# brech1/keaki

Hardware: AMD Instinct MI355X
Metric: BN254 G1 scalar-mults/sec on 2^24-point MSM (per GPU) (higher is better)
Workload: dtype u32 limbs, 256-bit Montgomery modular integer (9 x 29-bit lazy limbs in the bucket kernel, 8 x 32 elsewhere)

## Files before the change

keaki_amd/csrc/api.hip:

```cpp
#include "internal.h"

#include <algorithm>
#include <set>
#include <utility>
#include <vector>

using namespace keaki_internal;

struct keaki_hip_srs_g1 {
  const void* d = nullptr;
  size_t n = 0;
  bool owned = false;
  int device = -1;
  std::recursive_mutex mu;
  keaki_hip_ctx* acct = nullptr;
  size_t fk_bytes = 0;
  void* table = nullptr;
  size_t table_bytes = 0;
  int c_table = 0;
  void* fk_hat_s = nullptr;
  int fk_log2d = -1;
};
struct keaki_hip_srs_g2 {
  const void* d = nullptr;
// ... 295 lines not shown
    const size_t lo = pipe.ranges[j].first, m = pipe.ranges[j].second;
    return up.chunk(j, (char*)ctx->io_a.p + lo * 32, (const char*)scalars + lo * 32, m * 32);
  };
  return run(&pipe);
}

#define CTX_GUARD(ctx)                                \
  if (!(ctx)) return KEAKI_ERR_BAD_ARG;               \
  std::lock_guard<std::recursive_mutex> lock_((ctx)->mu);       \
  keaki_internal::DeviceScope dev_((ctx)->device);              \
  if (!dev_.ok) return fail(ctx, KEAKI_ERR_HIP, "hipSetDevice(%d) failed", (ctx)->device)

}

extern "C" {

#ifndef KEAKI_SRC_HASH
#define KEAKI_SRC_HASH "unknown"
#endif
#ifdef KEAKI_DIAG
const char* keaki_hip_version(void) { return "keaki-hip 0.3 (gfx950) DIAGNOSTIC BUILD (diag_row_mask available: not the product) src=" KEAKI_SRC_HASH; }
#else
const char* keaki_hip_version(void) { return "keaki-hip 0.3 (gfx950) src=" KEAKI_SRC_HASH; }
#endif

extern "C++" {
namespace {
void tune_from_env(Tuning& t) {
  auto geti = [](const char* name, long long& out) { const char* e = getenv(name); if (!e || !*e) return false; out = atoll(e); return true; };
  long long v;
  if (geti("KEAKI_MSM_C", v)) t.msm_c = (int)v;
  if (geti("KEAKI_MSM_C_SHARED", v)) t.msm_c_shared = (int)v;
  if (geti("KEAKI_REDUCE_L", v)) t.reduce_l = (int)v;
  if (geti("KEAKI_PART_SHIFT", v)) t.part_shift = (int)v;
  if (geti("KEAKI_ACC_U29", v)) t.acc_u29 = v != 0;
  if (geti("KEAKI_ACC_U29_G2", v)) t.acc_u29_g2 = v != 0;
  if (geti("KEAKI_ACC_NT", v)) t.acc_nt = v != 0;
  if (geti("KEAKI_ACC_PREFETCH", v)) t.acc_prefetch = v != 0;
  if (geti("KEAKI_ACC_IDXQ", v)) t.acc_idxq = v != 0;
  if (geti("KEAKI_CS_MASKED", v)) t.cs_masked = v != 0;
  if (geti("KEAKI_FK_UNIFORM", v)) t.fk_uniform = v != 0;
  if (geti("KEAKI_FK_GTAB", v)) t.fk_gtab = v != 0;
  if (geti("KEAKI_FK_ADDSUB29", v)) t.fk_addsub29 = v != 0;
  if (geti("KEAKI_FK_RADIX4", v)) t.fk_radix4 = v != 0;
  if (geti("KEAKI_FB_OCC1", v)) t.fb_occ1 = v != 0;
  if (geti("KEAKI_MSM_SHORT_TABLES", v)) t.msm_short_tables = (int)v;
  if (geti("KEAKI_PAIR_WIDE_MAX", v)) t.pair_wide_max = (int)v;
  if (geti("KEAKI_PAIR_TWO_WAVES", v)) t.pair_two_waves = v != 0;
  if (geti("KEAKI_GT_WB_B", v)) t.gt_wb_b = (int)v;
  if (geti("KEAKI_ENCAP_GT", v)) t.encap_gt = v;
  if (geti("KEAKI_HOST_PREFAULT", v)) t.host_prefault = v != 0;
  if (geti("KEAKI_PIPE_CHUNKS", v)) t.pipe_chunks = v != 0;
  if (geti("KEAKI_MSM_PIPE_CHUNKS", v)) t.msm_pipe_chunks = (int)v;
  if (geti("KEAKI_MSM_PIPE_MIN", v)) t.msm_pipe_min = v;
  if (geti("KEAKI_MSM_PIPE_GROWTH", v)) t.msm_pipe_growth = (int)v;
}
struct BufClass { DevBuf* b; int cls; };
std::vector<BufClass> all_bufs(keaki_hip_ctx* ctx) {
  std::vector<BufClass> v;
  for (DevBuf* b : {&ctx->digits, &ctx->hist, &ctx->offsets, &ctx->cursor, &ctx->sorted, &ctx->buckets, &ctx->acc29, &ctx->partials, &ctx->wsums, &ctx->bsums,
                    &ctx->tmp_a, &ctx->tmp_b, &ctx->tmp_c, &ctx->io_a, &ctx->io_b, &ctx->io_c, &ctx->io_d, &ctx->io_e, &ctx->perm, &ctx->heavy,
                    &ctx->pair_ws, &ctx->verify_io, &ctx->g2gen_lines, &ctx->fk_tab, &ctx->g2pow_lines, &ctx->g2pow_pts})
    v.push_back({b, 1});
  for (DevBuf* b : {&ctx->fb_bases, &ctx->fb_g1_gen, &ctx->fb_g2_gen, &ctx->fb_com, &ctx->fb_tau, &ctx->gt_tab_a, &ctx->gt_tab_b, &ctx->gt_base,
                    &ctx->fbs_g2_gen, &ctx->fbs_tau, &ctx->fbs_g1_gen})
    v.push_back({b, 2});
// ... 42 lines not shown
  for (const BufClass& bc : all_bufs(ctx))
    if (bc.b->p) (void)hipFree(bc.b->p);
  for (auto& e : ctx->ev) if (e) (void)hipEventDestroy(e);
  for (auto& e : ctx->fk_ev) if (e) (void)hipEventDestroy(e);
  for (auto& e : ctx->pipe_in) if (e) (void)hipEventDestroy(e);
  for (auto& e : ctx->pipe_done) if (e) (void)hipEventDestroy(e);
  for (auto& e : ctx->open_ev) if (e) (void)hipEventDestroy(e);
  if (ctx->copy_stream) { (void)hipStreamSynchronize(ctx->copy_stream); (void)hipStreamDestroy(ctx->copy_stream); }
  for (auto& e : ctx->aux_ev) if (e) (void)hipEventDestroy(e);
  if (ctx->aux_stream) { (void)hipStreamSynchronize(ctx->aux_stream); (void)hipStreamDestroy(ctx->aux_stream); }
  if (ctx->own_stream) (void)hipStreamDestroy(ctx->stream);
  }
  delete ctx;
}

const char* keaki_hip_last_error(const keaki_hip_ctx* ctx) {
  if (!ctx) return g_create_error.c_str();
  thread_local std::string copy;
  keaki_hip_ctx* c = const_cast<keaki_hip_ctx*>(ctx);
  std::lock_guard<std::recursive_mutex> lock_(c->mu);
  copy = c->err;
  return copy.c_str();
}

keaki_status keaki_hip_ctx_set_option(keaki_hip_ctx* ctx, const char* name, int64_t value) {
  if (!ctx) return KEAKI_ERR_BAD_ARG;
  std::lock_guard<std::recursive_mutex> lock_(ctx->mu);
  if (!name) return fail(ctx, KEAKI_ERR_BAD_ARG, "ctx_set_option: name is null");
  Tuning& t = ctx->tune;
  const std::string k(name);
  if (k == "msm_c") t.msm_c = (int)value;
  else if (k == "msm_c_shared") t.msm_c_shared = (int)value;
  else if (k == "reduce_l") t.reduce_l = (int)value;
  else if (k == "part_shift") t.part_shift = (int)value;
  else if (k == "acc_u29") t.acc_u29 = value != 0;
  else if (k == "acc_u29_g2") t.acc_u29_g2 = value != 0;
  else if (k == "acc_nt") t.acc_nt = value != 0;
  else if (k == "acc_prefetch") t.acc_prefetch = value != 0;
  else if (k == "acc_idxq") t.acc_idxq = value != 0;
  else if (k == "cs_masked") t.cs_masked = value != 0;
  else if (k == "fk_uniform") t.fk_uniform = value != 0;
  else if (k == "fk_gtab") t.fk_gtab = value != 0;
  else if (k == "fk_addsub29") t.fk_addsub29 = value != 0;
  else if (k == "fk_radix4") t.fk_radix4 = value != 0;
  else if (k == "fb_occ1") t.fb_occ1 = value != 0;
  else if (k == "msm_short_tables") t.msm_short_tables = (int)value;
  else if (k == "pair_wide_max") t.pair_wide_max = (int)value;
  else if (k == "pair_two_waves") t.pair_two_waves = value != 0;
  else if (k == "gt_wb_b") {
    if (value != 0 && (value < 8 || value > 22 || gt_table_powers((uint32_t)value) > 320)) return fail(ctx, KEAKI_ERR_BAD_ARG, "ctx_set_option: gt_wb_b = %lld out of range", (long long)value);
    if ((int)value != t.gt_wb_b) { ctx->gt_b_ready = false; ctx->gt_b_fallback = false; }
    t.gt_wb_b = (int)value;
  } else if (k == "encap_gt") t.encap_gt = value;
  else if (k == "host_prefault") t.host_prefault = value != 0;
  else if (k == "pipe_chunks") t.pipe_chunks = value != 0;
#ifdef KEAKI_DIAG
  else if (k == "diag_row_mask") t.diag_row_mask = (unsigned)value;
#endif
  else if (k == "msm_pipe_chunks") t.msm_pipe_chunks = (int)value;
  else if (k == "msm_pipe_min") t.msm_pipe_min = value;
  else if (k == "msm_pipe_growth") t.msm_pipe_growth = (int)value;
  else return fail(ctx, KEAKI_ERR_BAD_ARG, "ctx_set_option: unknown option '%s'", name);
  return KEAKI_OK;
}
keaki_status keaki_hip_debug_set_alloc_limit(keaki_hip_ctx* ctx, size_t bytes) {
  if (!ctx) return KEAKI_ERR_BAD_ARG;
// ... 1081 lines not shown
```

keaki_amd/csrc/internal.h:

```cpp
#pragma once
#include <hip/hip_runtime.h>

#include <cstdarg>
#include <cstdio>
#include <cstdlib>
#include <atomic>
#include <cstring>
#include <functional>
#include <mutex>
#include <string>
#include <utility>
#include <vector>

#include "../../include/keaki_hip.h"

namespace keaki_internal {

struct DevBuf {
  void* p = nullptr;
  size_t cap = 0;
};

}

namespace keaki_internal {
struct Tuning {
  int msm_c = 0;
  int msm_c_shared = 0;
  int msm_short_tables = -1;
  int reduce_l = 0;
  int part_shift = -1;
  bool acc_u29 = true;
  bool acc_u29_g2 = true;
  bool acc_prefetch = true;
  bool acc_idxq = true;
  bool cs_masked = true;
  bool acc_nt = false;
  bool fk_uniform = true;
  bool fk_gtab = true;
  bool fk_radix4 = true;
  bool fk_addsub29 = true;
  bool fb_occ1 = false;
  int pair_wide_max = -1;
  bool pair_two_waves = true;
  int gt_wb_b = 0;
  long long encap_gt = -1;
  bool host_prefault = true;
  bool pipe_chunks = true;
  int msm_pipe_chunks = -1;
  long long msm_pipe_min = 1 << 20;
  int msm_pipe_growth = 160;
#ifdef KEAKI_DIAG
  unsigned diag_row_mask = 0;
#endif
  size_t alloc_limit = 0;
};
}

struct keaki_hip_ctx {
  int device = 0;
  uint32_t n_cu = 256;
  keaki_internal::Tuning tune;
  std::atomic<size_t> mem_tables{0};
// ... 151 lines not shown
```

keaki_amd/csrc/msm.hip.h:

```cpp
#pragma once
#include <type_traits>
#include "bn254_curve.hip.h"
#include "fq29.hip.h"
#include "xyzz29.hip.h"
#include "jac29.hip.h"
#include "xyzz29_g2.hip.h"

namespace bn254 {

typedef uint16_t u16;
typedef u32 v4u_t __attribute__((ext_vector_type(4)));
constexpr u32 DIGIT_NONE = 0xFFFFFFFFu;
#ifndef STAMP
#define STAMP(cond, i) do { } while (0)
#endif

struct MsmShape {
  u32 n;
  u32 c;
  u32 W;
  u32 k;
  u32 stride;
};
KDEV u32 msm_width(const MsmShape& s, u32 w) { return w < s.k ? s.c : s.c - 1; }
// ... 1112 lines not shown
  }
  if (l == 0) {
    typename O::P r = sh[0];
    for (u32 k = 0, nd = msm_bit_offset(s, w); k < nd; k++) r = O::dbl(r);
    if (out_jac) store_norm_jac(out_jac, O::store(r));
    else window_sums[w] = O::store(r);
  }
}

template <class F> KDEV Aff<F> xyzz_to_aff_tail(const Xyzz<F>& p) { return xyzz_to_aff(p); }
template <> KDEV Aff<Fq> xyzz_to_aff_tail<Fq>(const Xyzz<Fq>& p) {
  if (xyzz_is_inf(p)) return aff_inf<Fq>();
  Fq izzz = fq_inv(p.zzz);
  Fq izz = fq_sqr(izzz) * fq_sqr(p.zz);
  return {p.x * izz, p.y * izzz};
}
template <class F>
KDEV void store_norm_jac(F* out, const Xyzz<F>& p) {
  Aff<F> a = xyzz_to_aff_tail(p);
  if (xyzz_is_inf(p)) {
    out[0] = f_one<F>(); out[1] = f_one<F>(); out[2] = f_zero<F>();
  } else {
    out[0] = a.x; out[1] = a.y; out[2] = f_one<F>();
  }
}
template <class F>
__global__ void __launch_bounds__(64) k_msm_final(const Xyzz<F>* __restrict__ window_sums, u32 W, F* __restrict__ out_jac) {
  if (threadIdx.x != 0 || blockIdx.x != 0) return;
  Xyzz<F> acc = xyzz_inf<F>();
  for (u32 w = 0; w < W; w++) acc = xyzz_add(acc, window_sums[w]);
  store_norm_jac(out_jac, acc);
}


template <class F>
__global__ void __launch_bounds__(64) k_msm_build_tables(const Aff<F>* __restrict__ points, u32 N, MsmShape s, Aff<F>* __restrict__ table) {
  u32 i = blockIdx.x * blockDim.x + threadIdx.x;
  if (i >= N) return;
  Aff<F> p = points[i];
  table[i] = p;
#pragma unroll 1
  for (u32 w = 1; w < s.W; w++) {
    Jac<F> j = jac_from_aff(p);
    for (u32 d = msm_width(s, w - 1); d > 0; d--) j = jac_dbl(j);
    p = jac_to_aff(j);
    table[(size_t)w * N + i] = p;
  }
}

constexpr u32 TABLE_MAX_W = 16;
static __global__ void __launch_bounds__(64) k_msm_build_tables_g1(const Aff<Fq>* __restrict__ points, u32 N, MsmShape s, Aff<Fq>* __restrict__ table) {
  u32 i = blockIdx.x * blockDim.x + threadIdx.x;
  if (i >= N) return;
  const Aff<Fq> p = points[i];
  table[i] = p;
  if (aff_is_inf(p)) {
    for (u32 w = 1; w < s.W; w++) table[(size_t)w * N + i] = p;
    return;
  }
  J29 j;
  j.x = u29_from_fq(p.x); j.y = u29_from_fq(p.y); j.z = u29_one();
  U29 zs[TABLE_MAX_W];
  U29 prod = u29_one();
#pragma unroll 1
  for (u32 w = 1; w < s.W; w++) {
    for (u32 d = msm_width(s, w - 1); d > 0; d--) j = j29_dbl(j);
// ... 39 lines not shown
```

keaki_amd/csrc/msm_host.hip.h:

```cpp
#pragma once
#include <algorithm>
#include <functional>
#include <type_traits>
#include <vector>
#include "internal.h"
#include "msm.hip.h"

namespace keaki_internal {
using namespace bn254;

inline int choose_window(size_t n, int forced = 0) {
  if (forced >= 3 && forced <= 24) return forced;
  if (n < 32) return 3;
  double best = 1e300;
  int bc = 3;
  for (int c = 3; c <= 22; c++) {
    MsmPlan p = msm_make_plan(n, c);
    if (p.nb > ((size_t)PART_MAX_BINS << PART_MAX_FINE_SHIFT)) continue;
    double cost = (double)n * p.s.W + 2.8 * (double)p.nb;
    if ((double)p.nb < 131072.0) cost *= 131072.0 / (double)p.nb;
    if (cost < best) { best = cost; bc = c; }
  }
  return bc;
}

template <class F>
keaki_status msm_dev(keaki_hip_ctx* ctx, const Aff<F>* d_points, size_t srs_len, const void* d_scalars, size_t n, void* d_out_jac,
                     const Aff<F>* d_table = nullptr, int c_table = 0, const MsmPipe* pipe = nullptr) {
  if (!d_out_jac || (n && (!d_points || !d_scalars))) return fail(ctx, KEAKI_ERR_BAD_ARG, "msm: null pointer");
  if (n > srs_len) return fail(ctx, KEAKI_ERR_TOO_LARGE, "msm: %zu scalars but the SRS holds %zu points", n, srs_len);
  if (n >= (1ull << 31)) return fail(ctx, KEAKI_ERR_BAD_ARG, "msm: n must be < 2^31 per device");
  const bool shared = d_table != nullptr && (n * 2 > srs_len || ctx->tune.msm_short_tables != 0);
  const MsmPlan plan = shared ? msm_make_plan(n, c_table) : msm_make_plan(n, choose_window(n, ctx->tune.msm_c));
  MsmShape s = plan.s;
  MsmShape rs = s;
  size_t nb = plan.nb;
  if (shared) {
    s.stride = (u32)srs_len;
    u32 cr = 0;
    while ((1u << cr) < plan.max_b) cr++;
    rs.n = s.n; rs.c = cr; rs.W = 1; rs.k = 1; rs.stride = 0;
    nb = plan.max_b;
    d_points = d_table;
    if ((double)srs_len * s.W >= 2147483647.0) return fail(ctx, KEAKI_ERR_BAD_ARG, "msm: precomputed table index overflows 31 bits");
  }
  ctx->last_c = (int)s.c;
  if ((double)n * s.W >= 4294967295.0) return fail(ctx, KEAKI_ERR_BAD_ARG, "msm: n * windows overflows 32-bit positions");
  u32 L = sizeof(F) > sizeof(Fq) ? (plan.max_b >= 64 ? 8 : plan.max_b)
                                 : plan.max_b >= (1u << 21) ? 32 : plan.max_b >= (1u << 20) ? 16 : (plan.max_b >= 64 ? 8 : plan.max_b);
  if (ctx->tune.reduce_l >= 1 && ctx->tune.reduce_l <= 4096 && (u32)ctx->tune.reduce_l <= plan.max_b) L = (u32)ctx->tune.reduce_l;
  const u32 chunks = cdiv(plan.max_b, L);
  ST_TRY(reserve(ctx, ctx->wsums, (size_t)rs.W * sizeof(Xyzz<F>)));
  Xyzz<F>* wsums = (Xyzz<F>*)ctx->wsums.p;
  F* out = (F*)d_out_jac;
  hipStream_t st = ctx->stream;
  if (ctx->timing) (void)hipEventRecord(ctx->ev[0], st);
  if (n == 0) {
    hipLaunchKernelGGL((k_msm_final<F>), dim3(1), dim3(64), 0, st, (const Xyzz<F>*)wsums, 0u, out);
    return launch_check(ctx, "msm_final");
  }
  const size_t K = pipe ? pipe->ranges.size() : 1;
  if (pipe && K < 1) return fail(ctx, KEAKI_ERR_BAD_ARG, "msm: bad chunk bounds");
  struct Pass {
    size_t lo, m, pairs, max_chunks, cm_bytes, bt_bytes, bm_bytes, sg_bytes, ts_bytes;
    PartShape ps;
  };
  std::vector<Pass> passes(K);
  size_t w_digits = 0, w_sorted = 0, w_offsets = 0, w_cursor = 0, w_pairs = 0, w_total = 0;
  for (size_t j = 0; j < K; j++) {
    Pass& q = passes[j];
    q.lo = pipe ? pipe->ranges[j].first : 0;
    q.m = pipe ? pipe->ranges[j].second : n;
    if (q.m == 0 || q.lo > n || q.m > n - q.lo) return fail(ctx, KEAKI_ERR_BAD_ARG, "msm: bad chunk bounds");
    w_total += q.m;
    if (!part_make_shape(q.m, s.W, nb, &q.ps, ctx->tune.part_shift))
      return fail(ctx, KEAKI_ERR_BAD_ARG, "msm: %zu buckets / %u windows exceed the bucket sort's LDS budget (window too large)", nb, s.W);
    q.pairs = q.m * (size_t)s.W;
    q.max_chunks = part_max_chunks(q.pairs, q.ps.nbins);
    q.cm_bytes = (size_t)q.ps.nbins * q.ps.ntiles * sizeof(uint2);
    q.bt_bytes = ((size_t)q.ps.nbins * 4 + 15) & ~(size_t)15;
    q.bm_bytes = (size_t)q.ps.nbins * sizeof(BinMeta);
    q.sg_bytes = nb * sizeof(v4u_t);
    q.ts_bytes = (size_t)q.ps.ntiles * (q.ps.nbins + 1) * 2;
    w_digits = std::max(w_digits, (size_t)q.ps.ntiles * q.ps.te * 4);
    w_sorted = std::max(w_sorted, q.pairs * 4 + 64);
    w_offsets = std::max(w_offsets, q.max_chunks * q.ps.nf * 4);
    w_cursor = std::max(w_cursor, q.cm_bytes + q.bt_bytes + q.bm_bytes + q.sg_bytes + q.ts_bytes);
    w_pairs = std::max(w_pairs, q.pairs);
  }
  if (w_total != n) return fail(ctx, KEAKI_ERR_BAD_ARG, "msm: the chunks cover %zu of %zu pairs", w_total, n);
  bool u29 = false;
  if constexpr (std::is_same<F, Fq>::value) u29 = ctx->tune.acc_u29;
  if constexpr (std::is_same<F, Fq2>::value) u29 = ctx->tune.acc_u29_g2;
  bool lazy_state = K > 1 && u29 && std::is_same<F, Fq>::value;
  ST_TRY(reserve(ctx, ctx->digits, w_digits));
  ST_TRY(reserve(ctx, ctx->sorted, w_sorted));
  ST_TRY(reserve(ctx, ctx->hist, nb * 4));
  ST_TRY(reserve(ctx, ctx->offsets, w_offsets));
  ST_TRY(reserve(ctx, ctx->cursor, w_cursor));
  ST_TRY(reserve(ctx, ctx->buckets, nb * sizeof(Xyzz<F>)));
  ST_TRY(reserve(ctx, ctx->partials, ((size_t)rs.W * chunks + (size_t)rs.W * 256) * sizeof(Xyzz<F>)));
  ST_TRY(reserve(ctx, ctx->perm, nb * 4 + 2 * CNT_BINS * 4 + sizeof(HeavyList)));
  const u32 hv_cap = (u32)(w_pairs / HEAVY_MIN + 1), hv_slice_cap = (u32)(hv_cap + w_pairs / HEAVY_SLICE + 1);
  const size_t hv_hdr = ((2 * (size_t)hv_cap + hv_slice_cap) * 4 + 255) & ~(size_t)255;
  ST_TRY(reserve(ctx, ctx->heavy, hv_hdr + (size_t)hv_slice_cap * sizeof(Xyzz<F>)));
  if (lazy_state) {
    const keaki_status st29 = reserve(ctx, ctx->acc29, nb * sizeof(Acc29));
    if (st29 == KEAKI_ERR_OOM) { lazy_state = false; u29 = false; ctx->err.clear(); }
    else if (st29 != KEAKI_OK) return st29;
  }
  u32 *tiles = (u32*)ctx->digits.p, *sorted = (u32*)ctx->sorted.p, *hist = (u32*)ctx->hist.p;
  u32* segoff = (u32*)ctx->offsets.p;
  Xyzz<F>* buckets = (Xyzz<F>*)ctx->buckets.p;
  Xyzz<F>* partials = (Xyzz<F>*)ctx->partials.p;
  Acc29* state29 = lazy_state ? (Acc29*)ctx->acc29.p : nullptr;
  u32* perm = (u32*)ctx->perm.p;
  u32 *gstart = perm + nb, *ghist = gstart + CNT_BINS;
  HeavyList* hv = (HeavyList*)(ghist + CNT_BINS);
  u32 *hv_bucket = (u32*)ctx->heavy.p, *hv_first = hv_bucket + hv_cap, *hv_owner = hv_first + hv_cap;
  Xyzz<F>* hv_slices = (Xyzz<F>*)((char*)ctx->heavy.p + hv_hdr);
  for (size_t j = 0; j < K; j++) {
    const Pass& q = passes[j];
    const PartShape& ps = q.ps;
    if (pipe && pipe->stage) ST_TRY(pipe->stage(j));
    MsmShape sj = s;
    sj.n = (u32)q.m;
    const Fr* scal = (const Fr*)d_scalars + q.lo;
    const Aff<F>* pts = d_points + q.lo;
    const bool first = j == 0, last = j + 1 == K;
    uint2* cellmeta = (uint2*)ctx->cursor.p;
    u32* bin_total = (u32*)((char*)ctx->cursor.p + q.cm_bytes);
    BinMeta* bins = (BinMeta*)((char*)bin_total + q.bt_bytes);
    v4u_t* segtab = (v4u_t*)((char*)bins + q.bm_bytes);
    u16* tstart = (u16*)((char*)segtab + q.sg_bytes);
// ... 48 lines not shown
        if (K == 1) {
          if (ctx->tune.acc_nt) KEAKI_ACC(1, ACC_WHOLE);
          else if (!ctx->tune.acc_prefetch)
            hipLaunchKernelGGL((k_msm_accumulate_g1_u29<0, ACC_WHOLE, 0>), ga, ba, 0, st, pts, view, (const u32*)hist, (const u32*)perm, (u32)nb, buckets, state29);
          else if (!ctx->tune.acc_idxq)
            hipLaunchKernelGGL((k_msm_accumulate_g1_u29<0, ACC_WHOLE, 1>), ga, ba, 0, st, pts, view, (const u32*)hist, (const u32*)perm, (u32)nb, buckets, state29);
          else KEAKI_ACC(0, ACC_WHOLE);
        }
        else if (first) KEAKI_ACC(0, ACC_FIRST);
        else if (!last) KEAKI_ACC(0, ACC_MIDDLE);
        else KEAKI_ACC(0, ACC_LAST);
#undef KEAKI_ACC
        done = true;
      }
    }
    if constexpr (std::is_same<F, Fq2>::value) {
      if (u29) {
        if (first) hipLaunchKernelGGL(k_msm_accumulate_g2_u29<0>, ga, ba, 0, st, pts, view, (const u32*)hist, (const u32*)perm, (u32)nb, buckets);
        else hipLaunchKernelGGL(k_msm_accumulate_g2_u29<1>, ga, ba, 0, st, pts, view, (const u32*)hist, (const u32*)perm, (u32)nb, buckets);
        done = true;
      }
    }
    if (!done)
      hipLaunchKernelGGL((k_msm_accumulate<F>), ga, ba, 0, st, pts, view, (const u32*)hist, (const u32*)perm, (u32)nb, buckets, first ? 0u : 1u);
    ST_TRY(launch_check(ctx, "msm_accumulate"));
    const u32 hv_mode = lazy_state && !last ? (first ? HV_SET29 : HV_ADD29) : (first ? HV_SET : HV_ADD);
    hipLaunchKernelGGL((k_msm_heavy<F>), dim3(HEAVY_GRID), dim3(256), 0, st, pts, view, (const u32*)hist,
                       (const HeavyList*)hv, hv_slice_cap, (const u32*)hv_bucket, (const u32*)hv_first, (const u32*)hv_owner, hv_slices);
    hipLaunchKernelGGL((k_msm_heavy_combine<F>), dim3(HEAVY_COMBINE_GRID), dim3(64), 0, st, (const u32*)hist, (const HeavyList*)hv, hv_cap, hv_slice_cap,
                       (const u32*)hv_bucket, (const u32*)hv_first, (const Xyzz<F>*)hv_slices, buckets, hv_mode, state29);
    ST_TRY(launch_check(ctx, "msm_heavy"));
  }
  if (ctx->timing) (void)hipEventRecord(ctx->ev[2], st);
  hipLaunchKernelGGL((k_msm_reduce<F>), dim3(cdiv((size_t)rs.W * chunks, 64)), dim3(64), 0, st, (const Xyzz<F>*)buckets, rs, L, chunks, partials);
  const Xyzz<F>* fin_in = partials;
  u32 fin_chunks = chunks;
  if (chunks > 256) {
    const u32 G = cdiv(chunks, 128);
    const u32 chunks2 = cdiv(chunks, G);
    Xyzz<F>* partials2 = partials + (size_t)rs.W * chunks;
    hipLaunchKernelGGL((k_msm_partial_groups<F>), dim3(chunks2, rs.W), dim3(64), 0, st, (const Xyzz<F>*)partials, chunks, G, chunks2, partials2);
    fin_in = partials2; fin_chunks = chunks2;
  }
  hipLaunchKernelGGL((k_msm_window_finish<F>), dim3(rs.W), dim3(64), 0, st, fin_in, rs, fin_chunks, wsums, rs.W == 1 ? out : (F*)nullptr);
  if (rs.W != 1) hipLaunchKernelGGL((k_msm_final<F>), dim3(1), dim3(64), 0, st, (const Xyzz<F>*)wsums, rs.W, out);
  ST_TRY(launch_check(ctx, "msm_reduce/final"));
  if (ctx->timing) {
    (void)hipEventRecord(ctx->ev[3], st);
    ctx->timing_pending = true;
  }
  return KEAKI_OK;
}

template <class F>
keaki_status msm_build_tables(keaki_hip_ctx* ctx, const Aff<F>* d_points, size_t N, int c_table, Aff<F>* d_table) {
  MsmPlan plan = msm_make_plan(N, c_table);
  bool done = false;
  if constexpr (std::is_same<F, Fq>::value) {
    if (plan.s.W <= TABLE_MAX_W) {
      hipLaunchKernelGGL(k_msm_build_tables_g1, dim3(cdiv(N, 64)), dim3(64), 0, ctx->stream, d_points, (u32)N, plan.s, d_table);
      done = true;
    }
  }
  if (!done)
  hipLaunchKernelGGL((k_msm_build_tables<F>), dim3(cdiv(N, 64)), dim3(64), 0, ctx->stream, d_points, (u32)N, plan.s, d_table);
  return launch_check(ctx, "msm_build_tables");
// ... 18 lines not shown
```

Baseline: 1.040 billion.

## Replace G1 MSM bucket reduction tail with hierarchical scan and cooperative final sum

Adds a new G1 MSM tail that replaces the per-window reduce, partial-group, window-finish and final kernels. Buckets are summed per chunk as running sums, combined in shared-memory tree groups into per-bit records, and then turned into weighted terms. The terms are doubled by window offset using an 8-lane cooperative XYZZ add/double, and the last block, chosen through an atomic counter, sums them into the output. The aim is to cut serial work and kernel launches in the tail and to spread the per-window doublings and final sum across many threads. The cost is more synchronisation, extra scratch memory, and a last-block reduction pattern that relies on threadfence ordering.

```diff
diff --git a/keaki_amd/csrc/api.hip b/keaki_amd/csrc/api.hip
--- a/keaki_amd/csrc/api.hip
+++ b/keaki_amd/csrc/api.hip
@@ -351,6 +351,7 @@
   if (geti("KEAKI_MSM_C", v)) t.msm_c = (int)v;
   if (geti("KEAKI_MSM_C_SHARED", v)) t.msm_c_shared = (int)v;
   if (geti("KEAKI_REDUCE_L", v)) t.reduce_l = (int)v;
+  if (geti("KEAKI_MSM_TAIL", v)) t.msm_tail = (int)v;
   if (geti("KEAKI_PART_SHIFT", v)) t.part_shift = (int)v;
   if (geti("KEAKI_ACC_U29", v)) t.acc_u29 = v != 0;
   if (geti("KEAKI_ACC_U29_G2", v)) t.acc_u29_g2 = v != 0;
@@ -459,6 +460,7 @@
   if (k == "msm_c") t.msm_c = (int)value;
   else if (k == "msm_c_shared") t.msm_c_shared = (int)value;
   else if (k == "reduce_l") t.reduce_l = (int)value;
+  else if (k == "msm_tail") t.msm_tail = (int)value;
   else if (k == "part_shift") t.part_shift = (int)value;
   else if (k == "acc_u29") t.acc_u29 = value != 0;
   else if (k == "acc_u29_g2") t.acc_u29_g2 = value != 0;
diff --git a/keaki_amd/csrc/internal.h b/keaki_amd/csrc/internal.h
--- a/keaki_amd/csrc/internal.h
+++ b/keaki_amd/csrc/internal.h
@@ -29,6 +29,7 @@
   int msm_c_shared = 0;
   int msm_short_tables = -1;
   int reduce_l = 0;
+  int msm_tail = 1;
   int part_shift = -1;
   bool acc_u29 = true;
   bool acc_u29_g2 = true;
diff --git a/keaki_amd/csrc/msm.hip.h b/keaki_amd/csrc/msm.hip.h
--- a/keaki_amd/csrc/msm.hip.h
+++ b/keaki_amd/csrc/msm.hip.h
@@ -1168,6 +1168,211 @@
   store_norm_jac(out_jac, acc);
 }
 
+constexpr u32 TAILW_SLOTS = 16;
+KDEV void x29w_add(bool act, u32 tl, const X29* A, const X29* B, X29* out, U29* scr) {
+  const bool both = act && !A->inf && !B->inf;
+  if (both && tl < 6) {
+    const U29& p = tl == 0 ? A->x : tl == 1 ? B->x : tl == 2 ? A->y : tl == 3 ? B->y : tl == 4 ? A->zz : A->zzz;
+    const U29& q = tl == 0 ? B->zz : tl == 1 ? A->zz : tl == 2 ? B->zzz : tl == 3 ? A->zzz : tl == 4 ? B->zz : B->zzz;
+    scr[tl] = u29_mul(p, q);
+  }
+  __syncthreads();
+  U29 P, R, U1;
+  bool slow = false;
+  if (both) {
+    U1 = scr[0];
+    P = u29_sub(scr[1], U1, Q29::K8);
+    R = u29_sub(scr[3], scr[2], Q29::K8);
+    slow = u29_maybe_zero(P) && u29_is_zero(P);
+    if (tl < 2) {
+      const U29 o = tl == 0 ? P : R;
+      scr[6 + tl] = u29_mul(o, o);
+    }
+  }
+  __syncthreads();
+  if (both && tl < 3) {
+    const U29 a = tl == 0 ? P : tl == 1 ? U1 : scr[4];
+    scr[8 + tl] = u29_mul(a, scr[6]);
+  }
+  __syncthreads();
+  U29 X3;
+  if (both) {
+    X3 = u29_sub3(scr[7], scr[8], scr[9]);
+    const U29 T = u29_sub_raw(scr[9], X3, Q29::K16);
+    if (tl < 3) {
+      const U29 a = tl == 0 ? scr[5] : tl == 1 ? scr[2] : R;
+      const U29 b = tl == 2 ? T : scr[8];
+      scr[11 + tl] = u29_mul(a, b);
+    }
+  }
+  __syncthreads();
+  if (act && tl == 0) {
+    X29 r;
+    if (A->inf) r = *B;
+    else if (B->inf) r = *A;
+    else if (slow) r = x29_add(*A, *B);
+    else {
+      r.x = X3;
+      r.y = u29_sub(scr[13], scr[12], Q29::K2);
+      r.zz = scr[10];
+      r.zzz = scr[11];
+      r.inf = 0;
+    }
+    *out = r;
+  }
+  __syncthreads();
+}
+KDEV void x29w_dbl(bool act, u32 tl, const X29* A, X29* out, U29* scr) {
+  const bool live = act && !A->inf;
+  U29 U;
+  if (live) {
+    U29 t;
+#pragma unroll
+    for (int i = 0; i < 9; i++) t.l[i] = A->y.l[i] << 1;
+    U = u29_carry(t);
+    if (tl < 2) {
+      const U29 o = tl == 0 ? U : A->x;
+      scr[tl] = u29_mul(o, o);
+    }
+  }
+  __syncthreads();
+  U29 M;
+  if (live) {
+    U29 t;
+#pragma unroll
+    for (int i = 0; i < 9; i++) t.l[i] = 3u * scr[1].l[i];
+    M = u29_carry(t);
+    if (tl < 4) {
+      const U29 a = tl == 0 ? U : tl == 1 ? A->x : tl == 2 ? M : scr[0];
+      const U29 b = tl == 2 ? M : tl == 3 ? A->zz : scr[0];
+      scr[2 + tl] = u29_mul(a, b);
+    }
+  }
+  __syncthreads();
+  U29 X3;
+  if (live) {
+    U29 t;
+#pragma unroll
+    for (int i = 0; i < 9; i++) t.l[i] = scr[4].l[i] - 2u * scr[3].l[i] + Q29::K16W[i];
+    X3 = u29_carry(t);
+    const U29 T = u29_sub_raw(scr[3], X3, Q29::K32);
+    if (tl < 3) {
+      const U29 a = tl == 0 ? M : scr[2];
+      const U29 b = tl == 0 ? T : tl == 1 ? A->y : A->zzz;
+      scr[6 + tl] = u29_mul(a, b);
+    }
+  }
+  __syncthreads();
+  if (act && tl == 0 && live) {
+    X29 r;
+    r.x = X3;
+    r.y = u29_sub(scr[6], scr[7], Q29::K4);
+    r.zz = scr[5];
+    r.zzz = scr[8];
+    r.inf = 0;
+    *out = r;
+  }
+  __syncthreads();
+}
+constexpr u32 TAIL_GROUP_BITS = 8;
+constexpr u32 TAIL_THREADS = 256;
+
+template <class F>
+__global__ void __launch_bounds__(64) k_msm_tail_chunks(const Xyzz<F>* __restrict__ buckets, MsmShape s, u32 lb, u32 chunks_per_window,
+                                                        Xyzz<F>* __restrict__ runs, Xyzz<F>* __restrict__ wss, u32* __restrict__ counter) {
+  const u32 g = blockIdx.x * blockDim.x + threadIdx.x;
+  if (g == 0) *counter = 0;
+  if (g >= s.W * chunks_per_window) return;
+  const u32 w = g / chunks_per_window, t = g % chunks_per_window;
+  const u32 L = 1u << lb, lo = t << lb;
+  const u32 Bw = msm_nbuckets(s, w);
+  const Xyzz<F>* bk = buckets + msm_bucket_base(s, w);
+  typedef TailOps<F> O;
+  typename O::P run = O::inf(), ws = O::inf();
+  for (u32 j = L; j-- > 0;) {
+    if (lo + j < Bw) {
+      run = O::add(run, O::load(bk[lo + j]));
+      ws = O::add(ws, run);
+    }
+  }
+  runs[g] = O::store(run);
+  wss[g] = O::store(ws);
+}
+
+template <class F>
+__global__ void __launch_bounds__(TAIL_THREADS) k_msm_tail_groups(const Xyzz<F>* __restrict__ runs, const Xyzz<F>* __restrict__ wss, u32 chunks_per_window,
+                                                                  u32 gb, Xyzz<F>* __restrict__ rec) {
+  typedef TailOps<F> O;
+  __shared__ typename O::P sh[2 * TAIL_THREADS];
+  const u32 w = blockIdx.y, x = blockIdx.x, l = threadIdx.x;
+  const u32 G = 1u << gb;
+  const size_t t0 = (size_t)w * chunks_per_window + ((size_t)x << gb);
+  if (l < G) {
+    sh[2 * l] = O::load(wss[t0 + l]);
+    sh[2 * l + 1] = O::load(runs[t0 + l]);
+  }
+  __syncthreads();
+  for (u32 d = 0; d < gb; d++) {
+    const u32 nn = G >> (d + 1), half = 1u << (d + 1);
+    const u32 nadd = nn * (d + 2);
+    typename O::P r = O::inf(), c = O::inf();
+    u32 slot = 0, cslot = 0;
+    if (l < nadd) {
+      const u32 k = l / nn, n = l % nn;
+      slot = (n << (d + 2)) + k;
+      r = O::add(sh[slot], sh[slot + half]);
+    }
+    if (l < nn) {
+      cslot = (l << (d + 2));
+      c = sh[cslot + half + 1];
+    }
+    __syncthreads();
+    if (l < nadd) sh[slot] = r;
+    if (l < nn) sh[cslot + d + 2] = c;
+    __syncthreads();
+  }
+  if (l < gb + 2) rec[((size_t)w * gridDim.x + x) * (gb + 2) + l] = O::store(sh[l]);
+}
+
+KDEV void tail_tree(X29* sh, U29* scr, u32 l) {
+  for (u32 h = TAIL_THREADS / 2; h > 8; h >>= 1) {
+    if (l < h) sh[l] = x29_add(sh[l], sh[l + h]);
+    __syncthreads();
+  }
+  const u32 team = l >> 3;
+  for (u32 h = 8; h > 0; h >>= 1) x29w_add(team < h, l & 7, sh + team, sh + team + h, sh + team, scr + (team < 8 ? team : 0) * TAILW_SLOTS);
+}
+
+static __global__ void __launch_bounds__(TAIL_THREADS) k_msm_tail_terms(const Xyzz<Fq>* __restrict__ rec, MsmShape s, u32 lb, u32 gb, u32 gpw,
+                                                                       Xyzz<Fq>* __restrict__ terms, u32* __restrict__ counter, Fq* __restrict__ out_jac) {
+  __shared__ X29 sh[TAIL_THREADS];
+  __shared__ U29 scr[8 * TAILW_SLOTS];
+  __shared__ u32 last;
+  const u32 o = blockIdx.x, w = blockIdx.y, l = threadIdx.x, nt = gridDim.x;
+  const u32 k = o == 0 ? 0u : o <= gb ? o + 1 : 1u;
+  X29 acc = x29_inf();
+  for (u32 x = l; x < gpw; x += TAIL_THREADS)
+    if (o <= gb || ((x >> (o - 1 - gb)) & 1)) acc = x29_add(acc, x29_load(rec[((size_t)w * gpw + x) * (gb + 2) + k]));
+  sh[l] = acc;
+  __syncthreads();
+  tail_tree(sh, scr, l);
+  for (u32 e = msm_bit_offset(s, w) + (o == 0 ? 0u : lb + o - 1); e > 0; e--) x29w_dbl(l < 8, l & 7, sh, sh, scr);
+  if (l == 0) {
+    terms[(size_t)w * nt + o] = x29_store(sh[0]);
+    __threadfence();
+    last = atomicAdd(counter, 1u) == nt * gridDim.y - 1 ? 1u : 0u;
+  }
+  __syncthreads();
+  if (!last) return;
+  __threadfence();
+  acc = x29_inf();
+  for (u32 i = l; i < nt * gridDim.y; i += TAIL_THREADS) acc = x29_add(acc, x29_load(terms[i]));
+  sh[l] = acc;
+  __syncthreads();
+  tail_tree(sh, scr, l);
+  if (l == 0) store_norm_jac(out_jac, x29_store(sh[0]));
+}
+
 
 template <class F>
 __global__ void __launch_bounds__(64) k_msm_build_tables(const Aff<F>* __restrict__ points, u32 N, MsmShape s, Aff<F>* __restrict__ table) {
diff --git a/keaki_amd/csrc/msm_host.hip.h b/keaki_amd/csrc/msm_host.hip.h
--- a/keaki_amd/csrc/msm_host.hip.h
+++ b/keaki_amd/csrc/msm_host.hip.h
@@ -22,6 +22,25 @@
     if (cost < best) { best = cost; bc = c; }
   }
   return bc;
+}
+
+struct TailShape {
+  u32 lb, cpw, gb, gpw, hb, nt;
+  size_t points(u32 W) const { return 2 * (size_t)W * cpw + (size_t)W * gpw * (gb + 2) + (size_t)W * nt + 1; }
+};
+inline TailShape tail_make_shape(u32 W, u32 max_b) {
+  TailShape t;
+  u32 mb = 1, lmb = 0;
+  while (mb < max_b) { mb <<= 1; lmb++; }
+  t.lb = 0;
+  while (t.lb < 4 && t.lb < lmb && (size_t)W * (mb >> t.lb) > (1u << 17)) t.lb++;
+  t.cpw = mb >> t.lb;
+  const u32 lc = lmb - t.lb;
+  t.gb = lc < TAIL_GROUP_BITS ? lc : TAIL_GROUP_BITS;
+  t.hb = lc - t.gb;
+  t.gpw = 1u << t.hb;
+  t.nt = 1 + t.gb + t.hb;
+  return t;
 }
 
 template <class F>
@@ -99,7 +118,9 @@
   ST_TRY(reserve(ctx, ctx->offsets, w_offsets));
   ST_TRY(reserve(ctx, ctx->cursor, w_cursor));
   ST_TRY(reserve(ctx, ctx->buckets, nb * sizeof(Xyzz<F>)));
-  ST_TRY(reserve(ctx, ctx->partials, ((size_t)rs.W * chunks + (size_t)rs.W * 256) * sizeof(Xyzz<F>)));
+  const bool new_tail = std::is_same<F, Fq>::value && ctx->tune.msm_tail != 0;
+  const TailShape ts = tail_make_shape(rs.W, plan.max_b);
+  ST_TRY(reserve(ctx, ctx->partials, std::max((size_t)rs.W * chunks + (size_t)rs.W * 256, new_tail ? ts.points(rs.W) : 0) * sizeof(Xyzz<F>)));
   ST_TRY(reserve(ctx, ctx->perm, nb * 4 + 2 * CNT_BINS * 4 + sizeof(HeavyList)));
   const u32 hv_cap = (u32)(w_pairs / HEAVY_MIN + 1), hv_slice_cap = (u32)(hv_cap + w_pairs / HEAVY_SLICE + 1);
   const size_t hv_hdr = ((2 * (size_t)hv_cap + hv_slice_cap) * 4 + 255) & ~(size_t)255;
@@ -214,6 +235,23 @@
     ST_TRY(launch_check(ctx, "msm_heavy"));
   }
   if (ctx->timing) (void)hipEventRecord(ctx->ev[2], st);
+  if constexpr (std::is_same<F, Fq>::value) if (new_tail) {
+    Xyzz<F>* runs = partials;
+    Xyzz<F>* wss = runs + (size_t)rs.W * ts.cpw;
+    Xyzz<F>* rec = wss + (size_t)rs.W * ts.cpw;
+    Xyzz<F>* terms = rec + (size_t)rs.W * ts.gpw * (ts.gb + 2);
+    u32* counter = (u32*)(terms + (size_t)rs.W * ts.nt);
+    hipLaunchKernelGGL((k_msm_tail_chunks<F>), dim3(cdiv((size_t)rs.W * ts.cpw, 64)), dim3(64), 0, st, (const Xyzz<F>*)buckets, rs, ts.lb, ts.cpw, runs, wss,
+                       counter);
+    hipLaunchKernelGGL((k_msm_tail_groups<F>), dim3(ts.gpw, rs.W), dim3(TAIL_THREADS), 0, st, (const Xyzz<F>*)runs, (const Xyzz<F>*)wss, ts.cpw, ts.gb, rec);
+    hipLaunchKernelGGL(k_msm_tail_terms, dim3(ts.nt, rs.W), dim3(TAIL_THREADS), 0, st, (const Xyzz<F>*)rec, rs, ts.lb, ts.gb, ts.gpw, terms, counter, out);
+    ST_TRY(launch_check(ctx, "msm_tail"));
+    if (ctx->timing) {
+      (void)hipEventRecord(ctx->ev[3], st);
+      ctx->timing_pending = true;
+    }
+    return KEAKI_OK;
+  }
   hipLaunchKernelGGL((k_msm_reduce<F>), dim3(cdiv((size_t)rs.W * chunks, 64)), dim3(64), 0, st, (const Xyzz<F>*)buckets, rs, L, chunks, partials);
   const Xyzz<F>* fin_in = partials;
   u32 fin_chunks = chunks;
```

Result: no change. 1.050 billion, median of 6 (+0.9%).

## Replace MSM bucket reduction tail with 2D row/column decomposition

Applied to the files above, without the earlier changes.

Replaces the running-sum bucket reduction (reduce, partial groups, window finish, final) with a three-kernel tail. Buckets are viewed as a 2D grid of H rows by K columns, where the bucket index j+1 splits into a high and a low part. Row and column strip sums are reduced into line sums, and these are combined by bit decomposition with doublings into per-window terms. The last block folds all terms into the output via an atomic counter, which exposes far more parallelism than sequential running sums. In exchange it adds extra point additions and doublings, a last-block-done synchronisation, and new code that is on by default (msm_tail=1).

```diff
diff --git a/keaki_amd/csrc/api.hip b/keaki_amd/csrc/api.hip
--- a/keaki_amd/csrc/api.hip
+++ b/keaki_amd/csrc/api.hip
@@ -351,6 +351,7 @@
   if (geti("KEAKI_MSM_C", v)) t.msm_c = (int)v;
   if (geti("KEAKI_MSM_C_SHARED", v)) t.msm_c_shared = (int)v;
   if (geti("KEAKI_REDUCE_L", v)) t.reduce_l = (int)v;
+  if (geti("KEAKI_MSM_TAIL", v)) t.msm_tail = (int)v;
   if (geti("KEAKI_PART_SHIFT", v)) t.part_shift = (int)v;
   if (geti("KEAKI_ACC_U29", v)) t.acc_u29 = v != 0;
   if (geti("KEAKI_ACC_U29_G2", v)) t.acc_u29_g2 = v != 0;
@@ -459,6 +460,7 @@
   if (k == "msm_c") t.msm_c = (int)value;
   else if (k == "msm_c_shared") t.msm_c_shared = (int)value;
   else if (k == "reduce_l") t.reduce_l = (int)value;
+  else if (k == "msm_tail") t.msm_tail = (int)value;
   else if (k == "part_shift") t.part_shift = (int)value;
   else if (k == "acc_u29") t.acc_u29 = value != 0;
   else if (k == "acc_u29_g2") t.acc_u29_g2 = value != 0;
diff --git a/keaki_amd/csrc/internal.h b/keaki_amd/csrc/internal.h
--- a/keaki_amd/csrc/internal.h
+++ b/keaki_amd/csrc/internal.h
@@ -29,6 +29,7 @@
   int msm_c_shared = 0;
   int msm_short_tables = -1;
   int reduce_l = 0;
+  int msm_tail = 1;
   int part_shift = -1;
   bool acc_u29 = true;
   bool acc_u29_g2 = true;
diff --git a/keaki_amd/csrc/models/model_tail.py b/keaki_amd/csrc/models/model_tail.py
--- /dev/null
+++ b/keaki_amd/csrc/models/model_tail.py
@@ -0,0 +1,150 @@
+#!/usr/bin/env python3
+
+R = 21888242871839275222246405745257275088548364400416034343698204186575808495617
+C = 12
+SLOTS = 256 * 4 * 3 * 64
+
+
+def tail_shape(max_b, W, n_cu=256):
+    cr = 0
+    while (1 << cr) < max_b:
+        cr += 1
+    kb = (cr + 1) // 2
+    m = 8
+    while True:
+        K = 1 << kb
+        H = -(-max_b // K)
+        SR, SC = -(-K // m), -(-H // m)
+        P1 = H * SR + K * SC
+        if W * P1 <= n_cu * 4 * 3 * 64 or m >= 4096:
+            break
+        m += 1
+    hb = 0
+    while (1 << hb) < H:
+        hb += 1
+    return kb, m, H, SR, SC, P1, hb, hb + kb + 1
+
+
+class Tally:
+    def __init__(self):
+        self.equal = 0
+        self.opposite = 0
+
+    def add(self, a, b, where=None, log=None):
+        if a and b:
+            if a == b:
+                self.equal += 1
+                if log is not None:
+                    log.append(("equal", where))
+            elif (a + b) % R == 0:
+                self.opposite += 1
+                if log is not None:
+                    log.append(("opposite", where))
+        return (a + b) % R
+
+
+def _tree(vals, t, where, log):
+    sh = list(vals)
+    q = len(sh) // 2
+    while q > 0:
+        for l in range(q):
+            sh[l] = t.add(sh[l], sh[l + q], where, log)
+        q //= 2
+    return sh[0]
+
+
+def window_terms(S, max_b, W, t, log=None, bit_offset=0):
+    kb, m, H, SR, SC, P1, hb, nU = tail_shape(max_b, W)
+    K, Bw = 1 << kb, len(S)
+    parts = []
+    for tt in range(P1):
+        if tt < H * SR:
+            l0 = (tt % SR) * m
+            j, step, cnt, kind = (tt // SR) * K + l0, 1, min(m, K - l0), "row"
+        else:
+            u = tt - H * SR
+            j, step, cnt, kind = (u // K) * m * K + u % K, K, m, "column"
+        acc = 0
+        i = 0
+        while i < cnt and j < Bw:
+            acc = t.add(acc, S[j], ("strip", kind), log)
+            i += 1
+            j += step
+        parts.append(acc)
+    lines = []
+    for o in range(H + K):
+        lane = [0] * 16
+        for l in range(16):
+            if o < H:
+                for s in range(l, SR, 16):
+                    lane[l] = t.add(lane[l], parts[o * SR + s], ("line", "row"), log)
+            else:
+                for s in range(l, SC, 16):
+                    lane[l] = t.add(lane[l], parts[H * SR + s * K + (o - H)], ("line", "column"), log)
+        lines.append(_tree(lane, t, ("line", "row" if o < H else "column"), log))
+    terms = []
+    for u in range(nU):
+        lane = [0] * 256
+        for l in range(256):
+            if u < hb:
+                for h in range(l, H, 256):
+                    if (h >> u) & 1:
+                        lane[l] = t.add(lane[l], lines[h], ("term", "row"), log)
+                shift = bit_offset + kb + u
+            else:
+                b = u - hb
+                for c in range(l, K, 256):
+                    if ((c + 1) >> b) & 1:
+                        lane[l] = t.add(lane[l], lines[H + c], ("term", "column"), log)
+                shift = bit_offset + b
+        v = _tree(lane, t, ("term", u), log)
+        for _ in range(shift):
+            v = t.add(v, v, ("double", u), log)
+        terms.append(v)
+    return terms, lines
+
+
+def tail(windows, max_b, bit_offsets, log=None):
+    t = Tally()
+    W = len(windows)
+    terms = []
+    for w, S in enumerate(windows):
+        tw, _ = window_terms(S, max_b, W, t, log, bit_offsets[w])
+        terms += tw
+    lane = [0] * 256
+    for l in range(256):
+        for i in range(l, len(terms), 256):
+            lane[l] = t.add(lane[l], terms[i], ("final",), log)
+    return _tree(lane, t, ("final",), log), t
+
+
+def direct(windows, bit_offsets):
+    return sum(pow(2, bit_offsets[w], R) * sum((j + 1) * s for j, s in enumerate(S)) for w, S in enumerate(windows)) % R
+
+
+A, B = 0x1234567, 0x89ABCDEF
+CASES = {
+    "strip_equal": [(A, 1), (A, 2)],
+    "column_opposite": [(A, 6), (R - A, 6 + 64)],
+    "row_identity": [(A, 129), (B, 130), (R - A - B, 191)],
+    "identity_result": [(A, 2), (R - 2 * A, 1)],
+}
+
+
+def case_inputs(name):
+    pairs = CASES[name]
+    return [d for d, _ in pairs], [k for _, k in pairs]
+
+
+def case_buckets(name, max_b=1 << (C - 1)):
+    S = [0] * max_b
+    for d, k in CASES[name]:
+        S[k - 1] = (S[k - 1] + d) % R
+    return S
+
+
+if __name__ == "__main__":
+    for name in sorted(CASES):
+        log = []
+        res, t = tail([case_buckets(name)], 1 << (C - 1), [0], log)
+        print(name, "result", res, "equal", t.equal, "opposite", t.opposite, sorted(set(log))[:6])
diff --git a/keaki_amd/csrc/msm.hip.h b/keaki_amd/csrc/msm.hip.h
--- a/keaki_amd/csrc/msm.hip.h
+++ b/keaki_amd/csrc/msm.hip.h
@@ -1168,6 +1168,118 @@
   store_norm_jac(out_jac, acc);
 }
 
+struct TailShape {
+  u32 kb;
+  u32 m;
+  u32 H;
+  u32 SR, SC;
+  u32 P1;
+  u32 hb;
+  u32 nU;
+};
+inline TailShape tail_make_shape(u32 max_b, u32 kb, u32 m) {
+  TailShape t;
+  t.kb = kb;
+  t.m = m;
+  const u32 K = 1u << kb;
+  t.H = (max_b + K - 1) / K;
+  t.SR = (K + m - 1) / m;
+  t.SC = (t.H + m - 1) / m;
+  t.P1 = t.H * t.SR + K * t.SC;
+  t.hb = 0;
+  while ((1u << t.hb) < t.H) t.hb++;
+  t.nU = t.hb + kb + 1;
+  return t;
+}
+template <class F>
+__global__ void __launch_bounds__(256) k_msm_tail_strips(const Xyzz<F>* __restrict__ buckets, MsmShape s, TailShape ts, Xyzz<F>* __restrict__ partials,
+                                                         u32* __restrict__ done) {
+  const u32 w = blockIdx.y, t = blockIdx.x * blockDim.x + threadIdx.x;
+  if (t == 0 && w == 0) *done = 0;
+  if (t >= ts.P1) return;
+  typedef TailOps<F> O;
+  const u32 K = 1u << ts.kb, Bw = msm_nbuckets(s, w), nr = ts.H * ts.SR;
+  const Xyzz<F>* bk = buckets + msm_bucket_base(s, w);
+  u32 j, step, cnt;
+  if (t < nr) {
+    const u32 l0 = (t % ts.SR) * ts.m;
+    j = (t / ts.SR) * K + l0; step = 1; cnt = min(ts.m, K - l0);
+  } else {
+    const u32 u = t - nr;
+    j = (u / K) * ts.m * K + u % K; step = K; cnt = ts.m;
+  }
+  typename O::P acc = O::inf();
+  for (u32 i = 0; i < cnt && j < Bw; i++, j += step) acc = O::add(acc, O::load(bk[j]));
+  partials[(size_t)w * ts.P1 + t] = O::store(acc);
+}
+template <class F>
+__global__ void __launch_bounds__(64) k_msm_tail_lines(const Xyzz<F>* __restrict__ partials, TailShape ts, Xyzz<F>* __restrict__ lines) {
+  typedef TailOps<F> O;
+  __shared__ typename O::P sh[64];
+  const u32 w = blockIdx.y, l = threadIdx.x, g = l & 15u, o = blockIdx.x * 4 + (l >> 4), K = 1u << ts.kb;
+  const Xyzz<F>* p = partials + (size_t)w * ts.P1;
+  typename O::P acc = O::inf();
+  if (o < ts.H) {
+    for (u32 t = g; t < ts.SR; t += 16) acc = O::add(acc, O::load(p[o * ts.SR + t]));
+  } else if (o < ts.H + K) {
+    for (u32 t = g; t < ts.SC; t += 16) acc = O::add(acc, O::load(p[ts.H * ts.SR + t * K + (o - ts.H)]));
+  }
+  sh[l] = acc;
+  __syncthreads();
+  for (u32 q = 8; q > 0; q >>= 1) {
+    if (g < q) sh[l] = O::add(sh[l], sh[l + q]);
+    __syncthreads();
+  }
+  if (g == 0 && o < ts.H + K) lines[(size_t)w * (ts.H + K) + o] = O::store(sh[l]);
+}
+template <class F>
+__global__ void __launch_bounds__(256) k_msm_tail_terms(const Xyzz<F>* __restrict__ lines, MsmShape s, TailShape ts, Xyzz<F>* __restrict__ terms,
+                                                        u32* __restrict__ done, F* __restrict__ out_jac) {
+  typedef TailOps<F> O;
+  __shared__ typename O::P sh[256];
+  __shared__ u32 last;
+  const u32 w = blockIdx.y, u = blockIdx.x, l = threadIdx.x, K = 1u << ts.kb;
+  const Xyzz<F>* ln = lines + (size_t)w * (ts.H + K);
+  typename O::P acc = O::inf();
+  u32 shift = msm_bit_offset(s, w);
+  if (u < ts.hb) {
+    for (u32 h = l; h < ts.H; h += 256)
+      if ((h >> u) & 1) acc = O::add(acc, O::load(ln[h]));
+    shift += ts.kb + u;
+  } else {
+    const u32 b = u - ts.hb;
+    for (u32 c = l; c < K; c += 256)
+      if (((c + 1) >> b) & 1) acc = O::add(acc, O::load(ln[ts.H + c]));
+    shift += b;
+  }
+  sh[l] = acc;
+  __syncthreads();
+  for (u32 q = 128; q > 0; q >>= 1) {
+    if (l < q) sh[l] = O::add(sh[l], sh[l + q]);
+    __syncthreads();
+  }
+  const u32 nt = gridDim.x * gridDim.y;
+  if (l == 0) {
+    typename O::P r = sh[0];
+    for (u32 i = 0; i < shift; i++) r = O::dbl(r);
+    terms[w * ts.nU + u] = O::store(r);
+    __threadfence();
+    last = atomicAdd(done, 1u) == nt - 1 ? 1u : 0u;
+  }
+  __syncthreads();
+  if (!last) return;
+  __threadfence();
+  acc = O::inf();
+  for (u32 i = l; i < nt; i += 256) acc = O::add(acc, O::load(terms[i]));
+  sh[l] = acc;
+  __syncthreads();
+  for (u32 q = 128; q > 0; q >>= 1) {
+    if (l < q) sh[l] = O::add(sh[l], sh[l + q]);
+    __syncthreads();
+  }
+  if (l == 0) store_norm_jac(out_jac, O::store(sh[0]));
+}
+
 
 template <class F>
 __global__ void __launch_bounds__(64) k_msm_build_tables(const Aff<F>* __restrict__ points, u32 N, MsmShape s, Aff<F>* __restrict__ table) {
diff --git a/keaki_amd/csrc/msm_host.hip.h b/keaki_amd/csrc/msm_host.hip.h
--- a/keaki_amd/csrc/msm_host.hip.h
+++ b/keaki_amd/csrc/msm_host.hip.h
@@ -50,6 +50,11 @@
                                  : plan.max_b >= (1u << 21) ? 32 : plan.max_b >= (1u << 20) ? 16 : (plan.max_b >= 64 ? 8 : plan.max_b);
   if (ctx->tune.reduce_l >= 1 && ctx->tune.reduce_l <= 4096 && (u32)ctx->tune.reduce_l <= plan.max_b) L = (u32)ctx->tune.reduce_l;
   const u32 chunks = cdiv(plan.max_b, L);
+  const bool new_tail = ctx->tune.msm_tail != 0;
+  u32 cr_all = 0;
+  while ((1u << cr_all) < plan.max_b) cr_all++;
+  TailShape ts = tail_make_shape(plan.max_b, (cr_all + 1) / 2, 8);
+  while ((size_t)rs.W * ts.P1 > (size_t)ctx->n_cu * 4 * 3 * 64 && ts.m < 4096) ts = tail_make_shape(plan.max_b, ts.kb, ts.m + 1);
   ST_TRY(reserve(ctx, ctx->wsums, (size_t)rs.W * sizeof(Xyzz<F>)));
   Xyzz<F>* wsums = (Xyzz<F>*)ctx->wsums.p;
   F* out = (F*)d_out_jac;
@@ -99,7 +104,8 @@
   ST_TRY(reserve(ctx, ctx->offsets, w_offsets));
   ST_TRY(reserve(ctx, ctx->cursor, w_cursor));
   ST_TRY(reserve(ctx, ctx->buckets, nb * sizeof(Xyzz<F>)));
-  ST_TRY(reserve(ctx, ctx->partials, ((size_t)rs.W * chunks + (size_t)rs.W * 256) * sizeof(Xyzz<F>)));
+  const size_t tail_pts = new_tail ? (size_t)rs.W * ((size_t)ts.P1 + ts.H + ((size_t)1 << ts.kb) + ts.nU) : (size_t)rs.W * chunks + (size_t)rs.W * 256;
+  ST_TRY(reserve(ctx, ctx->partials, tail_pts * sizeof(Xyzz<F>) + 64));
   ST_TRY(reserve(ctx, ctx->perm, nb * 4 + 2 * CNT_BINS * 4 + sizeof(HeavyList)));
   const u32 hv_cap = (u32)(w_pairs / HEAVY_MIN + 1), hv_slice_cap = (u32)(hv_cap + w_pairs / HEAVY_SLICE + 1);
   const size_t hv_hdr = ((2 * (size_t)hv_cap + hv_slice_cap) * 4 + 255) & ~(size_t)255;
@@ -214,6 +220,20 @@
     ST_TRY(launch_check(ctx, "msm_heavy"));
   }
   if (ctx->timing) (void)hipEventRecord(ctx->ev[2], st);
+  if (new_tail) {
+    Xyzz<F>* lines = partials + (size_t)rs.W * ts.P1;
+    Xyzz<F>* terms = lines + (size_t)rs.W * (ts.H + ((size_t)1 << ts.kb));
+    u32* done = (u32*)(terms + (size_t)rs.W * ts.nU);
+    hipLaunchKernelGGL((k_msm_tail_strips<F>), dim3(cdiv(ts.P1, 256), rs.W), dim3(256), 0, st, (const Xyzz<F>*)buckets, rs, ts, partials, done);
+    hipLaunchKernelGGL((k_msm_tail_lines<F>), dim3(cdiv(ts.H + ((size_t)1 << ts.kb), 4), rs.W), dim3(64), 0, st, (const Xyzz<F>*)partials, ts, lines);
+    hipLaunchKernelGGL((k_msm_tail_terms<F>), dim3(ts.nU, rs.W), dim3(256), 0, st, (const Xyzz<F>*)lines, rs, ts, terms, done, out);
+    ST_TRY(launch_check(ctx, "msm_tail"));
+    if (ctx->timing) {
+      (void)hipEventRecord(ctx->ev[3], st);
+      ctx->timing_pending = true;
+    }
+    return KEAKI_OK;
+  }
   hipLaunchKernelGGL((k_msm_reduce<F>), dim3(cdiv((size_t)rs.W * chunks, 64)), dim3(64), 0, st, (const Xyzz<F>*)buckets, rs, L, chunks, partials);
   const Xyzz<F>* fin_in = partials;
   u32 fin_chunks = chunks;
```

Result: no change. 1.050 billion before, 1.054 billion after, median of 6 (+0.3%).
